# rrwick/Polypolish

Hardware: NVIDIA H100
Metric: assembly Mbp polished/sec (higher is better)
Workload: dtype u8 bases / u32 counters / f64 depth

## Files before the change

polypolish_b200/csrc/polish_dev.cuh:

```cuda
#pragma once

#include "nib_utils.h"
#include "../../include/pp_abi.h"

#define PP_BIN_SHIFT 8
#define PP_BIN (1u << PP_BIN_SHIFT)
#define PP_SUB_SHIFT 7
#define PP_SUB (1u << PP_SUB_SHIFT)
#define TL_T 2048
#define TL_THREADS 512
#define TL_PER_THREAD (TL_T / TL_THREADS)
#define TL_LONG_E 512
#define TL_QCAP 1024
#define TL_FAST_LEN 192
#define PR_THREADS 256
#define SC_GROUP_SCAN_LIMIT 8192
#define VT_THREADS 256
#define VT_ITEMS 8
#define VT_CHUNK (VT_THREADS * VT_ITEMS)
#define NONE32 0xFFFFFFFFu
static_assert(VT_CHUNK == TL_T, "k_tile hands k_compact one chunk per tile");
static_assert(TL_T % PP_BIN == 0 && TL_T / PP_SUB == TL_THREADS / 32 && TL_PER_THREAD * 32 == PP_SUB, "tile = whole bins; warp w owns depth sub-tile w and votes on it");

enum : unsigned {
    ERR_UNKNOWN_CONTIG = 1, ERR_SEQ_MISMATCH = 2, ERR_BAD_OP = 3, ERR_OOB = 4, ERR_NOSEQ = 5
};
enum : unsigned { FL_NODE_OVF = 1, FL_OUT_OVF = 8, FL_BIGGROUP = 16 };
enum : unsigned { TR_RC = 1, TR_FAST = 2, TR_LONG = 4, TR_FAST1 = 8 };

struct DevStatus {
    unsigned long long err;
    unsigned long long n_used;
    unsigned long long out_len;
    unsigned int node_count;
    unsigned int flags;
    unsigned int max_ext;
    unsigned int ticket;
    unsigned int n_changes;
    unsigned int pad1;
#ifdef PP_TILE_PROF
    unsigned long long prof[12];
#endif
};

struct DevParams {
    double fv, fi;
    uint32_t min_depth, max_errors;
    int careful;
    int pad;
};

struct OthNode {
    unsigned long long sig;
    unsigned long long val;
    uint32_t count;
    uint32_t next;
};

struct __align__(16) TileRec {
    uint32_t gstart;
    uint32_t seq_off;
    uint32_t cigar_off;
    uint32_t len_nc;
    uint32_t aln;
    uint32_t E;
    uint32_t flags;
    uint32_t cend;
};
#define TL_SEQ_QUADS 6

struct DevData {
    unsigned long long n_aln;
    const uint32_t *contig, *ref_start, *read_id, *seq_off, *cigar_off, *nm, *cigar_ops;
    const uint16_t *seq_len, *n_cigar;
// ... 575 lines not shown
    o.packed |= status << 26;
    if (vp.dbg) debug_record(vp.dbg + pos, depth, vt, it, cA, cC, cG, cT, cDel, matched, n_other, orig, status, o);
    if (CHG && status == 5) {
        const uint32_t slot = atomicAdd(vp.chg_n, 1u);
        if (slot < vp.chg_cap) {
            vp.chg_pos[slot] = pos;
            debug_record(vp.chg + slot, depth, vt, it, cA, cC, cG, cT, cDel, matched, n_other, orig, status, o);
        }
    }
    return o;
}

#define TL_DN_HALO 32
#define TL_INV_K 32
#define TL_DN_WORDS ((TL_T + 2 * TL_DN_HALO) / 16)

struct WalkStage {
    uint4 ent[64];
    uint32_t key[2][32];
};

#define TL_STAGES 2
struct ChunkStage {
    uint4 seq[32 * TL_SEQ_QUADS];
    TileRec rec[32];
};

#if defined(PP_EMULATE)
static inline void stage_bar_init(unsigned long long* bar) { emu::ring_init(bar); }
static inline void stage_fence() {}
static inline void stage_expect(unsigned long long* bar, uint32_t bytes) { emu::ring_expect(bar, bytes); }
static inline void stage_copy(void* dst, const void* src, uint32_t bytes, unsigned long long* bar) { emu::ring_copy(dst, src, bytes, bar); }
static inline void stage_wait(unsigned long long* bar, uint32_t parity) { emu::ring_wait(bar, parity); }
#else
__device__ __forceinline__ uint32_t smem_addr(const void* p) { return (uint32_t)__cvta_generic_to_shared(p); }
__device__ __forceinline__ void stage_bar_init(unsigned long long* bar) {
    asm volatile("mbarrier.init.shared::cta.b64 [%0], 1;\n\tfence.mbarrier_init.release.cluster;" ::"r"(smem_addr(bar)) : "memory");
}
__device__ __forceinline__ void stage_fence() { asm volatile("fence.proxy.async.shared::cta;" ::: "memory"); }
__device__ __forceinline__ void stage_expect(unsigned long long* bar, uint32_t bytes) {
    asm volatile("mbarrier.arrive.expect_tx.shared::cta.b64 _, [%0], %1;" ::"r"(smem_addr(bar)), "r"(bytes) : "memory");
}
__device__ __forceinline__ void stage_copy(void* dst, const void* src, uint32_t bytes, unsigned long long* bar) {
    asm volatile("cp.async.bulk.shared::cluster.global.mbarrier::complete_tx::bytes [%0], [%1], %2, [%3];"
                 ::"r"(smem_addr(dst)), "l"(src), "r"(bytes), "r"(smem_addr(bar)) : "memory");
}
__device__ __forceinline__ void stage_wait(unsigned long long* bar, uint32_t parity) {
    uint32_t done;
    do {
        asm volatile("{\n\t.reg .pred p;\n\tmbarrier.try_wait.parity.shared::cta.b64 p, [%1], %2;\n\tselp.u32 %0, 1, 0, p;\n\t}"
                     : "=r"(done) : "r"(smem_addr(bar)), "r"(parity) : "memory");
    } while (!done);
}
#endif

struct TileShared {
    int cdiff[TL_T + 4];
    uint32_t ex[4][TL_T];
    uint32_t del[TL_T];
    uint32_t oth[TL_T];
    union {
        unsigned long long deficit[TL_T + 4];
        double depth[TL_T];
    };
    unsigned long long dn[TL_DN_WORDS + 2];
    union {
        WalkStage wstage[TL_THREADS / 32];
        ChunkStage ring[TL_THREADS / 32][TL_STAGES];
    };
    unsigned long long ring_bar[TL_THREADS / 32][TL_STAGES];
    uint2 queue[TL_QCAP];
    uint32_t qn;
    unsigned long long s_warp[TL_THREADS / 32];
    unsigned long long s_total;
    long long s_delta[TL_THREADS / 32];
    uint32_t tile;
    uint32_t any_multi;
    double inv_k[TL_INV_K + 1];
    unsigned long long def_k[TL_INV_K + 1];
};
static_assert(sizeof(TileShared) <= 232448, "k_tile's shared memory: at most 227 KB per CTA on sm_90");

template <int BITS> struct TileCtx {
    const DevData& d;
    TileShared& sh;
    uint32_t P0;

    __device__ __forceinline__ bool in_tile(uint32_t pos) const { return pos - P0 < (uint32_t)TL_T; }
    __device__ __forceinline__ uint32_t draft_sym(uint32_t pos) const {
        if (BITS == 4) {
            const uint32_t o = pos - P0 + TL_DN_HALO;
            return (uint32_t)(sh.dn[o >> 4] >> ((o & 15) * 4)) & 15u;
        }
        const uint32_t b = d.draft[pos];
        return b == '-' ? 0u : b;
    }
    __device__ __forceinline__ void push_other(uint32_t pos, unsigned long long aln, uint32_t start, uint32_t len, unsigned long long sig) {
        if (!in_tile(pos)) return;
        atomicAdd(&sh.oth[pos - P0], 1u);
        other_insert<BITS>(d, pos, (aln << 32) | ((unsigned long long)(start & 0xFFFFu) << 16) | (len & 0xFFFFu), sig);
    }
    __device__ __forceinline__ void count_base(uint32_t pos, uint32_t s, unsigned long long aln, uint32_t ri) {
        if (!in_tile(pos)) return;
        if (Seq<BITS>::is_del(s)) { atomicAdd(&sh.del[pos - P0], 1u); return; }
        const uint32_t ds = draft_sym(pos);
// ... 18 lines not shown
    }
    __device__ __forceinline__ void scan_mismatches(unsigned long long r0, unsigned long long r1, uint32_t vc, uint32_t pos0,
                                                    unsigned long long aln, uint32_t ri0) {
        const long long rel64 = (long long)pos0 - (long long)P0;
        if (rel64 <= -32 || rel64 >= (long long)TL_T) return;
        const int rel0 = (int)rel64;
        unsigned long long d0, d1;
        draft32(rel0, d0, d1);
        unsigned long long m0, m1;
        mismatch_masks(r0, r1, d0, d1, vc, m0, m1);
        const int lo = -rel0, hi = TL_T - rel0;
        m0 &= nibmask(hi) & ~nibmask(lo);
        m1 &= nibmask(hi - 16) & ~nibmask(lo - 16);
        while (m0) {
            const uint32_t j = (uint32_t)(__ffsll((long long)m0) - 1) >> 2;
            m0 &= m0 - 1;
            const uint32_t code = (uint32_t)(r0 >> (4 * j)) & 15u;
            const int c = Seq<4>::acgt(code);
            if (c >= 0) atomicAdd(&sh.ex[c][rel0 + (int)j], 1u);
            else push_other(pos0 + j, aln, ri0 + j, 1, 1ull | ((unsigned long long)code << 4));
        }
        while (m1) {
            const uint32_t j = (uint32_t)(__ffsll((long long)m1) - 1) >> 2;
            m1 &= m1 - 1;
            const uint32_t code = (uint32_t)(r1 >> (4 * j)) & 15u;
            const int c = Seq<4>::acgt(code);
            if (c >= 0) atomicAdd(&sh.ex[c][rel0 + 16 + (int)j], 1u);
            else push_other(pos0 + 16 + j, aln, ri0 + 16 + j, 1, 1ull | ((unsigned long long)code << 4));
        }
    }
};

template <int BITS>
__device__ uint32_t general_walk(TileCtx<BITS>& S, const TileRec& r, uint32_t k) {
    const DevData& d = S.d;
    const unsigned long long aln = r.aln;
    const uint32_t len = r.len_nc & 0xFFFFu, ncig = r.len_nc >> 16;
    const bool rc = r.flags & TR_RC;
    const uint32_t gstart = r.gstart;
    const uint8_t* seqp = d.seq_pool + (size_t)r.seq_off * (BITS == 4 ? 16 : 32);
    const uint32_t* ops = d.cigar_ops + r.cigar_off;
    unsigned long long E = 0;
    for (uint32_t p = 0; p < ncig; ++p) {
        const uint32_t op = ops[p], o = op & 15u, l = op >> 4;
        if (o != PP_OP_I) E += l;
    }
    const uint32_t last = Seq<BITS>::read_sym(seqp, 0, len, rc, len - 1);
    unsigned long long run = 0;
    {
        uint32_t ri = len;
        uint32_t pend = 0;
        bool stop = false;
        for (int p = (int)ncig - 1; p >= 0 && !stop; --p) {
            const uint32_t op = ops[p], o = op & 15u, l = op >> 4;
            if (o == PP_OP_I) { pend += l; ri -= l; continue; }
            if (o == PP_OP_D) {
                for (uint32_t t = 0; t < l; ++t) {
                    if (pend == 1 && Seq<BITS>::read_sym(seqp, 0, len, rc, ri) == last) { run++; pend = 0; }
                    else { stop = true; break; }
                }
                continue;
            }
            for (uint32_t t = 0; t < l; ++t) {
                if (pend == 0 && Seq<BITS>::read_sym(seqp, 0, len, rc, ri - 1) == last) { run++; ri--; }
                else { stop = true; break; }
            }
        }
    }
    const unsigned long long nk64 = (E - run >= 1) ? (E - run - 1) : 0;
    if ((unsigned long long)gstart + nk64 > r.cend) { report_error(d.st, aln, ERR_OOB); return 0; }
    const uint32_t nkept = (uint32_t)nk64;
    S.add_interval(gstart, nkept, k);
    const long long off = (long long)S.P0 - (long long)gstart;
    const unsigned long long e_lo = off > 0 ? (unsigned long long)off : 0ull;
    const unsigned long long e_hi = min((unsigned long long)nkept, (unsigned long long)max(off + (long long)TL_T, 0ll));
    if (e_lo >= e_hi) return nkept;
    unsigned long long e = 0;
    uint32_t ri = 0;
    for (uint32_t p = 0; p < ncig && e < e_hi; ++p) {
        const uint32_t op = ops[p], o = op & 15u, l = op >> 4;
        if (o == PP_OP_I) { ri += l; continue; }
        uint32_t ins = 0;
        for (uint32_t q = p + 1; q < ncig && (ops[q] & 15u) == PP_OP_I; ++q) ins += ops[q] >> 4;
        const unsigned long long plain64 = min((unsigned long long)(ins ? l - 1 : l), (unsigned long long)nkept - e);
        const unsigned long long t_lo = e_lo > e ? e_lo - e : 0ull, t_hi = min(plain64, e_hi > e ? e_hi - e : 0ull);
        if (o == PP_OP_D) {
            for (unsigned long long t = t_lo; t < t_hi; ++t) atomicAdd(&S.sh.del[(uint32_t)(gstart + e + t) - S.P0], 1u);
            if (ins && e + l - 1 < nkept) {
                const uint32_t pos = (uint32_t)(gstart + e + l - 1);
                if (ins == 1) S.count_base(pos, Seq<BITS>::read_sym(seqp, 0, len, rc, ri), aln, ri);
                else S.push_other(pos, aln, ri, ins, make_sig<BITS>(seqp, 0, len, rc, ri, ins));
            }
            e += l;
            continue;
        }
        if (BITS == 4) {
            for (unsigned long long c0 = t_lo & ~31ull; c0 < t_hi; c0 += 32) {
                unsigned long long r0, r1;
                load_read32(reinterpret_cast<const unsigned long long*>(seqp), len, rc, ri + (uint32_t)c0, r0, r1);
                S.scan_mismatches(r0, r1, (uint32_t)min(plain64 - c0, 32ull), (uint32_t)(gstart + e + c0), aln, ri + (uint32_t)c0);
            }
        } else {
            for (unsigned long long t = t_lo; t < t_hi; ++t)
                S.count_base((uint32_t)(gstart + e + t), Seq<BITS>::read_sym(seqp, 0, len, rc, ri + (uint32_t)t), aln, ri + (uint32_t)t);
        }
        if (ins && e + l - 1 < nkept)
            S.push_other((uint32_t)(gstart + e + l - 1), aln, ri + l - 1, 1 + ins, make_sig<BITS>(seqp, 0, len, rc, ri + l - 1, 1 + ins));
        e += l;
        ri += l;
    }
    return nkept;
}

__device__ __forceinline__ uint32_t fast_walk(TileCtx<4>& S, const TileRec& r, const uint32_t* w, uint32_t k) {
    const uint32_t len = r.len_nc & 0xFFFFu;
    const unsigned long long aln = r.aln;
    if (len < 8) return NONE32;
    uint32_t run;
    const uint32_t tw = (len - 8) >> 3;
    const uint32_t tw0 = w[tw], tw1 = w[tw + 1];
    {
        const uint32_t o = len - 8;
        const uint32_t t8 = __funnelshift_r(tw0, tw1, (o & 7) * 4);
        const uint32_t x = t8 ^ ((t8 >> 28) * 0x11111111u);
        const uint32_t nz = (x | (x >> 1) | (x >> 2) | (x >> 3)) & 0x11111111u;
        if (nz == 0) return NONE32;
        run = 7u - ((31u - (uint32_t)__clz((int)nz)) >> 2);
    }
    const bool one = r.flags & TR_FAST1;
    const uint32_t ia = (r.flags >> 8) & 0xFFu, ib = (r.flags >> 16) & 0xFFFu;
    const bool is_del = (r.flags >> 28) & 1u;
    const uint32_t lc = len - ia - (is_del ? 0u : ib);
    if (run > lc) return NONE32;
    const uint32_t E = is_del ? len + ib : len - ib;
    const uint32_t nkept = E - run - 1;
    if ((unsigned long long)r.gstart + nkept > r.cend) { report_error(S.d.st, aln, ERR_OOB); return 0; }
    S.add_interval(r.gstart, nkept, k);
    const long long g0 = (long long)r.gstart - (long long)S.P0;
    if (g0 >= (long long)TL_T || g0 + (long long)nkept <= 0) return nkept;
    const uint32_t* dn32 = reinterpret_cast<const uint32_t*>(S.sh.dn);
    int relq[2], lo[2], hi[2], i0[2];
    uint32_t sh4[2], inner[2], edge[2];
    relq[0] = (int)g0;
    relq[1] = (int)g0 + (is_del ? (int)ib : -(int)ib);
    lo[0] = 0;
    hi[0] = !one ? (int)nkept : (int)ia - (is_del ? 0 : 1);
// ... 45 lines not shown
            const int rel = rq + 8 * (int)m + (int)t;
            if ((code & (code - 1)) == 0) atomicAdd(&S.sh.ex[__ffs((int)code) - 1][rel], 1u);
            else S.push_other(S.P0 + (uint32_t)rel, aln, 8u * m + t, 1, 1ull | ((unsigned long long)code << 4));
        }
    };
    uint32_t mm = (bits & cmp) | ((inner[0] | inner[1]) & ~cmp) | edge[0] | edge[1];
    {
        const bool sb = hi[1] > lo[1];
        const int e_lo = sb ? lo[1] : lo[0], e_hi = sb ? hi[1] : hi[0];
        const uint32_t m_last = (uint32_t)(e_hi - 1) >> 3;
        if (e_hi > e_lo && (((sb ? edge[1] : edge[0]) >> m_last) & 1u) && m_last - tw < 2u && (!sb || hi[0] <= 8 * (int)m_last)) {
            mm &= ~(1u << m_last);
            count_word(sb ? 1 : 0, m_last, m_last == tw ? tw0 : tw1);
        }
    }
    while (mm) {
        const uint32_t m = (uint32_t)__ffs((int)mm) - 1;
        mm &= mm - 1;
        const uint32_t wv = w[m];
        count_word(0, m, wv);
        if (one) count_word(1, m, wv);
    }
    if (one) {
        if (!is_del) {
            if (ia - 1 < nkept)
                S.push_other(r.gstart + ia - 1, aln, ia - 1, 1 + ib, make_sig<4>(S.d.seq_pool, r.seq_off, len, r.flags & TR_RC, ia - 1, 1 + ib));
        } else {
            const long long t0 = g0 + (long long)ia;
            const long long t_lo = max(0ll, -t0), t_hi = min((long long)min(ib, nkept - ia), (long long)TL_T - t0);
            for (long long t = t_lo; t < t_hi; ++t) atomicAdd(&S.sh.del[(int)(t0 + t)], 1u);
        }
    }
    return nkept;
}

__device__ __forceinline__ TileRec load_srec(const DevData& d, uint32_t slot) {
    const uint4* src = reinterpret_cast<const uint4*>(d.srec + slot);
    const uint4 a = __ldg(src), b = __ldg(src + 1);
    TileRec r;
    r.gstart = a.x; r.seq_off = a.y; r.cigar_off = a.z; r.len_nc = a.w; r.aln = b.x; r.E = b.y; r.flags = b.z; r.cend = b.w;
    return r;
}

#define DW_RUNS 4
#if defined(PP_EMULATE)
#define PP_PREFETCH_L1(p) ((void)(p))
#define PP_PREFETCH_L2(p) ((void)(p))
#else
#define PP_PREFETCH_L1(p) asm volatile("prefetch.global.L1 [%0];" ::"l"(p))
#define PP_PREFETCH_L2(p) asm volatile("prefetch.global.L2 [%0];" ::"l"(p))
#endif
template <int BITS>
__device__ void depth_walk_steps(const DevData& d, TileShared& sh, uint32_t P0, uint32_t sub, uint32_t lb, uint32_t long_lo, uint32_t long_hi) {
    const uint32_t lane = threadIdx.x & 31;
    const uint32_t s = P0 + sub * PP_SUB;
    const uint32_t bin = s >> PP_BIN_SHIFT;
    uint32_t wb[DW_RUNS], end[DW_RUNS], mask[DW_RUNS], head[DW_RUNS];
    uint32_t w_aln[DW_RUNS], w_start[DW_RUNS], w_len[DW_RUNS];
    double w_inv[DW_RUNS];
    auto load_window = [&](int r) {
        for (;;) {
            if (wb[r] >= end[r]) { mask[r] = 0; head[r] = NONE32; return; }
            const uint32_t slot = wb[r] + lane;
            uint4 q = make_uint4(NONE32, 0, 0, 1);
            if (slot < end[r]) {
                q = d.wrec[slot];
                if (slot + 32 < end[r]) PP_PREFETCH_L1(d.wrec + slot + 32);
            }
            uint32_t len = q.z;
            if (r == DW_RUNS - 1 && slot < end[r]) {
                const TileRec rec = load_srec(d, slot);
                const unsigned long long e_end = (unsigned long long)rec.gstart + rec.E;
                const uint32_t kk = d.kf[rec.aln];
                const bool mine = kk != 0 && e_end > P0 && rec.gstart < P0 + (uint32_t)TL_T;
                q.x = rec.aln; q.y = rec.gstart; q.w = mine ? kk : 1u;
                len = mine ? q.z : 0u;
// ... 122 lines not shown
    }
    double* out = sh.depth + (p - P0);
    out[0] = dep0; out[1] = dep1; out[2] = dep2; out[3] = dep3;
}

template <int BITS>
__device__ __forceinline__ void depth_walk(const DevData& d, TileShared& sh, WalkStage& ws, uint32_t P0, uint32_t sub, uint32_t lb, uint32_t long_lo, uint32_t long_hi) {
    const uint32_t bin = (P0 + sub * PP_SUB) >> PP_BIN_SHIFT;
    if (lb <= 1 && long_lo >= long_hi) {
        const uint32_t lo1 = d.bin_start[bin], hi1 = d.bin_start[bin + 1];
        uint32_t lo0 = 0, hi0 = 0;
        if (lb == 1 && bin >= 1) { lo0 = d.bin_start[bin - 1]; hi0 = lo1; }
        depth_walk_two<BITS>(d, sh, ws, P0, sub, lo0, hi0, lo1, hi1);
    } else depth_walk_steps<BITS>(d, sh, P0, sub, lb, long_lo, long_hi);
}

template <int BITS, bool CHG = false>
__device__ __forceinline__ void tile_body(const DevData& d, const VoteParams& vp, TileShared& sh) {
    const uint32_t tid = threadIdx.x, lane = tid & 31, warp = tid >> 5;
    const DevParams prm = *d.prm;
    const uint32_t lb = (d.max_ext + PP_BIN - 1) >> PP_BIN_SHIFT;
    const uint32_t long_lo = d.bin_start[d.n_bins], long_hi = d.bin_start[d.n_bins + 1];
    OthCtx oc;
    oc.nodes = d.nodes; oc.head = d.oth_head;
    oc.sr = SeqRef{d.seq_pool, d.seq_off, d.seq_len, d.flags};

    if (tid <= (uint32_t)TL_INV_K) {
        sh.inv_k[tid] = tid ? __ddiv_rn(1.0, (double)tid) : 0.0;
        sh.def_k[tid] = tid > 1 ? depth_deficit(tid) : 0ull;
    }
    ChunkStage* const ring = sh.ring[warp];
    unsigned long long* const bar = sh.ring_bar[warp];
    if (lane == 0) { stage_bar_init(&bar[0]); stage_bar_init(&bar[1]); }
    uint32_t parity = 0;
    for (;;) {
        stage_fence();
        __syncthreads();
        if (tid == 0) { sh.tile = atomicAdd(&d.st->ticket, 1u); sh.any_multi = 0; sh.qn = 0; }
        __syncthreads();
        if (sh.tile >= d.n_tiles) break;
        const uint32_t tile = d.tile_order[sh.tile];
        const uint32_t P0 = tile * (uint32_t)TL_T;
        TileCtx<BITS> S{d, sh, P0};
#ifdef PP_TILE_PROF
        long long pt[6];
        pt[0] = clock64();
#endif
        const uint32_t b0 = P0 >> PP_BIN_SHIFT;
        const uint32_t lo = d.bin_start[b0 >= lb ? b0 - lb : 0u];
        const uint32_t hi = d.bin_start[min(b0 + (uint32_t)(TL_T / PP_BIN), d.n_bins)];
        const uint32_t stride = 32u * (TL_THREADS / 32);
        uint32_t c_a = lo + 32u * warp;
        auto issue = [&](uint32_t c, uint32_t s) {
            const uint32_t n = min(32u, hi - c);
            stage_expect(&bar[s], n * (uint32_t)(sizeof(TileRec) + (BITS == 4 ? 16 * TL_SEQ_QUADS : 0)));
            stage_copy(ring[s].rec, d.srec + c, n * (uint32_t)sizeof(TileRec), &bar[s]);
            if (BITS == 4) stage_copy(ring[s].seq, d.sseq + (size_t)c * TL_SEQ_QUADS, n * 16u * TL_SEQ_QUADS, &bar[s]);
        };
        if (lane == 0) {
            if (c_a < hi) issue(c_a, 0);
            if (c_a + stride < hi) issue(c_a + stride, 1);
        }
        const uint32_t last_slot = d.n_slots ? d.n_slots - 1 : 0u;
        uint32_t k_a = 0;
        const uint32_t aln_a = __ldg(&d.srec[min(c_a + lane, last_slot)].aln);
        uint32_t aln_b = __ldg(&d.srec[min(c_a + stride + lane, last_slot)].aln);
        {
            uint4* z = reinterpret_cast<uint4*>(sh.cdiff);
            const uint32_t nz = (uint32_t)((size_t)((char*)sh.dn - (char*)sh.cdiff) / 16);
            for (uint32_t i = tid; i < nz; i += TL_THREADS) z[i] = make_uint4(0, 0, 0, 0);
            static_assert(TL_T == 4 * TL_THREADS, "one 16-byte store of chain heads per thread");
// ... 24 lines not shown
#ifdef PP_TILE_PROF
            unsigned long long wait_cyc = 0;
#endif
            uint32_t s = 0;
            while (c_a < hi) {
                const uint32_t c_b = c_a + stride, c_c = c_b + stride;
                uint32_t k_b = 0;
                if (c_b + lane < hi) k_b = d.kf[aln_b];
                const uint32_t aln_c = __ldg(&d.srec[min(c_c + lane, last_slot)].aln);
#ifdef PP_TILE_PROF
                const long long w0 = clock64();
#endif
                stage_wait(&bar[s], (parity >> s) & 1u);
                parity ^= 1u << s;
#ifdef PP_TILE_PROF
                if (lane == 0) wait_cyc += (unsigned long long)(clock64() - w0);
#endif
                const TileRec rec_a = ring[s].rec[lane];
                const uint32_t* const seq_a = reinterpret_cast<const uint32_t*>(ring[s].seq + lane * TL_SEQ_QUADS);
                const uint32_t i = c_a + lane;
                bool defer = false;
                if (i < hi) {
                    if (k_a == 0) d.wrec[i] = make_uint4(rec_a.aln, rec_a.gstart, 0u, 1u);
                    else {
                        uint32_t nk = NONE32;
                        if (BITS == 4 && (rec_a.flags & TR_FAST)) nk = fast_walk(reinterpret_cast<TileCtx<4>&>(S), rec_a, seq_a, k_a);
                        if (nk == NONE32) defer = true;
                        else d.wrec[i] = make_uint4(rec_a.aln, rec_a.gstart, nk, k_a);
                    }
                }
                if (defer) {
                    const uint32_t qi = atomicAdd(&sh.qn, 1u);
                    if (qi < TL_QCAP) {
                        sh.queue[qi] = make_uint2(i, k_a);
                        PP_PREFETCH_L2(d.cigar_ops + rec_a.cigar_off);
                        PP_PREFETCH_L2(d.seq_pool + (size_t)rec_a.seq_off * (BITS == 4 ? 16 : 32));
                    } else
                        d.wrec[i] = make_uint4(rec_a.aln, rec_a.gstart, general_walk<BITS>(S, rec_a, k_a), k_a);
                }
                __syncwarp();
                if (lane == 0 && c_c < hi) issue(c_c, s);
                c_a = c_b; aln_b = aln_c; k_a = k_b; s ^= 1u;
            }
#ifdef PP_TILE_PROF
            if (lane == 0 && wait_cyc) atomicAdd(&d.st->prof[11], wait_cyc);
#endif
        }
        __syncthreads();
#ifdef PP_TILE_PROF
        pt[2] = clock64();
#endif
        {
            const uint32_t qn = min(sh.qn, (uint32_t)TL_QCAP);
            for (uint32_t qi = lane * (TL_THREADS / 32) + warp; qi < qn; qi += TL_THREADS) {
                const uint2 q = sh.queue[qi];
                const TileRec r = load_srec(d, q.x);
                d.wrec[q.x] = make_uint4(r.aln, r.gstart, general_walk<BITS>(S, r, q.y), q.y);
            }
            for (uint32_t i = long_lo + tid; i < long_hi; i += TL_THREADS) {
                const TileRec r = load_srec(d, i);
                const unsigned long long e_end = (unsigned long long)r.gstart + r.E;
                const uint32_t k = d.kf[r.aln];
                if (k != 0 && e_end > P0 && r.gstart < P0 + (uint32_t)TL_T) d.wrec[i] = make_uint4(r.aln, r.gstart, general_walk<BITS>(S, r, k), k);
            }
        }
        __syncwarp();
        __syncthreads();
#ifdef PP_TILE_PROF
        pt[3] = clock64();
#endif
        const uint32_t rel0 = tid * TL_PER_THREAD;
        uint32_t cover[TL_PER_THREAD];
        uint32_t multi = 0;
        {
            long long csum = 0;
#pragma unroll
            for (int i = 0; i < TL_PER_THREAD; ++i) { csum += sh.cdiff[rel0 + i]; cover[i] = (uint32_t)csum; }
            const unsigned long long ex = block_exscan<TL_THREADS>((unsigned long long)csum, sh.s_warp, &sh.s_total);
#pragma unroll
            for (int i = 0; i < TL_PER_THREAD; ++i) cover[i] += (uint32_t)ex;
            if (sh.any_multi) {
                unsigned long long dsum = 0, dv[TL_PER_THREAD];
#pragma unroll
                for (int i = 0; i < TL_PER_THREAD; ++i) { dsum += sh.deficit[rel0 + i]; dv[i] = dsum; }
                const unsigned long long dex = block_exscan<TL_THREADS>(dsum, sh.s_warp, &sh.s_total);
#pragma unroll
                for (int i = 0; i < TL_PER_THREAD; ++i) {
                    sh.deficit[rel0 + i] = dv[i] + dex;
                    if (dv[i] + dex != 0 || cover[i] >= TL_DEF_COVER) multi |= 1u << i;
                }
            }
// ... 114 lines not shown
            if (n_zero) atomicAdd(&vp.zero_depth[ctg], (unsigned long long)n_zero);
            if (tdepth != 0.0) atomicAdd(&vp.total_depth[ctg], tdepth);
        }
        {
            uint32_t w2[TL_PER_THREAD / 2];
#pragma unroll
            for (int i = 0; i < TL_PER_THREAD; ++i) {
                const uint32_t len = po[i].packed & 0xFFFFu;
                uint32_t h;
                if ((po[i].packed >> 25) & 1u) { h = 255u << 8; if (p0 + i < d.G) vp.rec_at[p0 + i] = po[i].rec; }
                else h = (len << 8) | ((po[i].packed >> 16) & 255u);
                if (i & 1) w2[i >> 1] |= h << 16; else w2[i >> 1] = h;
            }
            *reinterpret_cast<uint2*>(vp.res + p0) = make_uint2(w2[0], w2[1]);
        }
        const uint32_t npos = (p0 < d.G) ? min((uint32_t)TL_PER_THREAD, d.G - p0) : 0u;
        long long delta = (long long)tlen - (long long)npos;
        for (int o = 16; o > 0; o >>= 1) delta += __shfl_down_sync(0xffffffffu, delta, o);
        if (lane == 0) sh.s_delta[warp] = delta;
#ifdef PP_TILE_PROF
        if (__syncthreads_or(walk) && tid == 0) atomicAdd(&d.st->prof[10], 1ull);
#endif
        __syncthreads();
        if (tid == 0) {
            long long t = 0;
            for (int i = 0; i < TL_THREADS / 32; ++i) t += sh.s_delta[i];
            vp.chunk_delta[tile] = t;
#ifdef PP_TILE_PROF
            pt[5] = clock64();
            for (int i = 0; i < 5; ++i) atomicAdd(&d.st->prof[i], (unsigned long long)(pt[i + 1] - pt[i]));
            atomicAdd(&d.st->prof[5], (unsigned long long)sh.qn);
            atomicAdd(&d.st->prof[6], 1ull);
            atomicMax(&d.st->prof[7], (unsigned long long)sh.qn);
#endif
        }
    }
}
static_assert(TL_PER_THREAD == 4, "the verdict store packs four positions per thread");

#if !defined(PP_EMULATE)
template <int BITS, bool CHG>
__global__ void __launch_bounds__(TL_THREADS, 1) k_tile(DevData d, VoteParams vp) {
    extern __shared__ __align__(16) unsigned char tile_smem[];
    tile_body<BITS, CHG>(d, vp, *reinterpret_cast<TileShared*>(tile_smem));
}
#endif

__device__ __forceinline__ uint8_t* put_u32(uint8_t* w, uint32_t v) {
    w[0] = (uint8_t)v; w[1] = (uint8_t)(v >> 8); w[2] = (uint8_t)(v >> 16); w[3] = (uint8_t)(v >> 24);
    return w + 4;
}
template <int BITS>
__device__ void allele_strings_row(const OthCtx& oc, uint32_t pos, uint32_t new_node, uint8_t* pool, unsigned long long cap,
                                   unsigned long long* used, unsigned long long* off) {
    unsigned long long bytes = 8;
    uint32_t n = 0;
    for (uint32_t nd = oc.head[pos]; nd != 0; nd = oc.nodes[nd - 1].next == NONE32 ? 0 : oc.nodes[nd - 1].next + 1) {
        bytes += 8 + ((uint32_t)oc.nodes[nd - 1].val & 0xFFFFu);
        n++;
    }
    const uint32_t new_len = new_node == NONE32 ? 0u : (uint32_t)oc.nodes[new_node].val & 0xFFFFu;
    bytes += new_len;
    const unsigned long long o = atomicAdd(used, bytes);
    *off = o;
    if (o + bytes > cap) return;
    uint8_t* w = put_u32(pool + o, n);
// ... 126 lines not shown
```

polypolish_b200/csrc/polish_kernels.cu:

```cuda
#include <cuda_runtime.h>

#include <cub/device/device_radix_sort.cuh>
#include <cub/device/device_scan.cuh>

#include <algorithm>
#include <functional>
#include <cstddef>
#include <cstdio>
#include <string>
#include <vector>

#include "pp_internal.h"
#include "pp_ctx.cuh"
#include "polish_dev.cuh"


static void init_comp_table(uint8_t* t) {
    for (int i = 0; i < 256; ++i) t[i] = 'N';
    const char* a = "ATGCNRYSWKMBVDH.-?";
    const char* b = "TACGNYRSWMKVBHD.-?";
    for (int i = 0; a[i]; ++i) t[(unsigned char)a[i]] = (uint8_t)b[i];
}

extern "C" const char* pp_version(void) { return "0.6.1-b200"; }
// ... 399 lines not shown
        vp.res = ctx->b[B_RES].as<uint16_t>(); vp.rec_at = ctx->b[B_RECAT].as<uint32_t>();
        vp.chunk_delta = ctx->b[B_CHUNKDELTA].as<long long>();
        vp.dbg = nullptr;
        if (ctx->debug_on) { CK(ctx->b[B_DEBUG].ensure((G + 1) * sizeof(pp_debug_pos))); vp.dbg = ctx->b[B_DEBUG].as<pp_debug_pos>(); }
        vp.chg = nullptr; vp.chg_pos = nullptr; vp.chg_n = &d.st->n_changes; vp.chg_cap = 0;
        if (ctx->changes_on) {
            if (ctx->chg_cap == 0) ctx->chg_cap = (uint32_t)std::max<uint64_t>(4096, G / 256);
            CK(ctx->b[B_CHG].ensure((size_t)ctx->chg_cap * sizeof(pp_debug_pos))); CK(ctx->b[B_CHGPOS].ensure((size_t)ctx->chg_cap * 4));
            vp.chg = ctx->b[B_CHG].as<pp_debug_pos>(); vp.chg_pos = ctx->b[B_CHGPOS].as<uint32_t>(); vp.chg_cap = ctx->chg_cap;
        }
        {
            int occ = 1;
            CK(cudaOccupancyMaxActiveBlocksPerMultiprocessor(&occ, vp.chg ? k_tile<BITS, true> : k_tile<BITS, false>, TL_THREADS, sizeof(TileShared)));
            const uint32_t grid = std::min<uint32_t>(n_tiles, (uint32_t)ctx->sm_count * (uint32_t)std::max(occ, 1));
            if (vp.chg) k_tile<BITS, true><<<grid, TL_THREADS, sizeof(TileShared), s>>>(d, vp);
            else k_tile<BITS, false><<<grid, TL_THREADS, sizeof(TileShared), s>>>(d, vp);
            ctx->launches++;
        }
        CK(cudaEventRecord(ctx->ev[4], s));
        k_compact<BITS><<<n_tiles, VT_THREADS, 0, s>>>(d, vp);
        ctx->launches++;
        CK(cudaEventRecord(ctx->ev[5], s));
        CK(cudaMemcpyAsync(ctx->h_status, d.st, sizeof(DevStatus), cudaMemcpyDeviceToHost, s));
        CK(cudaStreamSynchronize(s));
        CK(cudaGetLastError());
        const DevStatus hs = *ctx->h_status;
#ifdef PP_TILE_PROF
        fprintf(stderr, "[tile prof] tiles %llu; cycles/tile: A %.0f B %.0f queue %.0f C %.0f D+E %.0f; queued reads/tile %.1f (max %llu); "
                "chunk wait/tile/warp %.0f\n", hs.prof[6],
                (double)hs.prof[0] / hs.prof[6], (double)hs.prof[1] / hs.prof[6], (double)hs.prof[2] / hs.prof[6], (double)hs.prof[3] / hs.prof[6],
                (double)hs.prof[4] / hs.prof[6], (double)hs.prof[5] / hs.prof[6], hs.prof[7], (double)hs.prof[11] / hs.prof[6] / (TL_THREADS / 32));
        fprintf(stderr, "[tile prof] depth walks %llu (%.2f per tile, %llu tiles with one), %.0f cycles each\n", hs.prof[9], (double)hs.prof[9] / hs.prof[6], hs.prof[10],
                hs.prof[9] ? (double)hs.prof[8] / hs.prof[9] : 0.0);
#endif
        if (hs.err != ~0ull) {
            res->error_aln = (int64_t)(hs.err >> 8);
            return ctx->fail(PP_ERR_INPUT, std::string(err_text((unsigned)(hs.err & 0xFF))) + " (alignment " + std::to_string(hs.err >> 8) + ")");
        }
        bool again = false;
        if (hs.flags & FL_BIGGROUP) { if (ctx->global_k) return ctx->fail(PP_ERR_CUDA, "internal error: FL_BIGGROUP in global-k mode"); ctx->global_k = true; again = true; }
        if (hs.flags & FL_NODE_OVF) { ctx->node_cap = (uint32_t)std::min<uint64_t>(0x7FFFFFFFull, (uint64_t)hs.node_count + hs.node_count / 4 + 1024); again = true; }
        if (!again && (hs.flags & FL_OUT_OVF)) { ctx->out_cap = hs.out_len + 64; again = true; }
        if (!again && ctx->changes_on && hs.n_changes > ctx->chg_cap) { ctx->chg_cap = hs.n_changes; again = true; }
        if (again) continue;

        ctx->have_debug = ctx->debug_on; ctx->last_head = d.oth_head; ctx->last_nodes = std::min(hs.node_count, node_cap);
        ctx->have_changes = ctx->changes_on; ctx->n_changes = ctx->changes_on ? hs.n_changes : 0; ctx->chg_pool = -1;
        res->out_len = hs.out_len;
        res->n_aln_used = hs.n_used;
        res->error_aln = -1;
        memset(&res->timing, 0, sizeof res->timing);
        float ms;
        CK(cudaEventElapsedTime(&ms, ctx->ev[0], ctx->ev[1])); res->timing.stage_ms[0] = ms;
        CK(cudaEventElapsedTime(&ms, ctx->ev[1], ctx->ev[2])); res->timing.stage_ms[1] = ms;
        CK(cudaEventElapsedTime(&ms, ctx->ev[2], ctx->ev[3])); res->timing.stage_ms[2] = ms;
        CK(cudaEventElapsedTime(&ms, ctx->ev[3], ctx->ev[4])); res->timing.stage_ms[3] = ms;
        CK(cudaEventElapsedTime(&ms, ctx->ev[4], ctx->ev[5])); res->timing.stage_ms[4] = ms;
        CK(cudaEventElapsedTime(&ms, ctx->ev[0], ctx->ev[5])); res->timing.total_ms = ms;
        res->timing.launches = ctx->launches;

        if (res->out_bases) {
            if (res->out_cap < hs.out_len) return ctx->fail(PP_ERR_ARG, "out_cap too small: need " + std::to_string(hs.out_len) + " bytes");
            CK(cudaEventRecord(ctx->ev[7], s));
            CK(cudaMemcpyAsync(res->out_bases, vp.out, hs.out_len, cudaMemcpyDeviceToHost, s));
            if (res->out_off) CK(cudaMemcpyAsync(res->out_off, vp.out_off, ((size_t)ctx->n_contigs + 1) * 8, cudaMemcpyDeviceToHost, s));
            if (res->changed) CK(cudaMemcpyAsync(res->changed, vp.changed, (size_t)ctx->n_contigs * 8, cudaMemcpyDeviceToHost, s));
// ... 172 lines not shown
```

Before: 8319.

## Drain deferred-read queue with early-finishing warps and stage walks in shared memory

Warps that finish the chunk loop early now pull deferred reads from a shared work queue using CAS and acquire loads while other warps are still busy, instead of waiting at the barrier. Each queued walk copies the read's sequence and CIGAR into the warp's free ring buffer in shared memory before lane 0 walks it, which cuts global-memory latency during the serial walk. This adds spin-wait and nanosleep overhead, a fence, and more atomics on shared memory. It also adds extra profiling counters.

```diff
diff --git a/polypolish_b200/csrc/polish_dev.cuh b/polypolish_b200/csrc/polish_dev.cuh
--- a/polypolish_b200/csrc/polish_dev.cuh
+++ b/polypolish_b200/csrc/polish_dev.cuh
@@ -39,7 +39,7 @@
     unsigned int n_changes;
     unsigned int pad1;
 #ifdef PP_TILE_PROF
-    unsigned long long prof[12];
+    unsigned long long prof[17];
 #endif
 };
 
@@ -681,7 +681,14 @@
 static inline void stage_expect(unsigned long long* bar, uint32_t bytes) { emu::ring_expect(bar, bytes); }
 static inline void stage_copy(void* dst, const void* src, uint32_t bytes, unsigned long long* bar) { emu::ring_copy(dst, src, bytes, bar); }
 static inline void stage_wait(unsigned long long* bar, uint32_t parity) { emu::ring_wait(bar, parity); }
+template <class V> static inline V ld_acquire_cta(const V* p) { return __atomic_load_n(p, __ATOMIC_ACQUIRE); }
+static inline void st_relaxed_cta(unsigned long long* p, unsigned long long v) { __atomic_store_n(p, v, __ATOMIC_RELAXED); }
+static inline void fence_cta() { std::atomic_thread_fence(std::memory_order_seq_cst); }
+static inline void backoff(unsigned ns) { std::this_thread::sleep_for(std::chrono::nanoseconds(ns)); }
+static std::atomic<unsigned long long> emu_queue_walks[3];
+#define EMU_QUEUE_COUNT(i, n) emu_queue_walks[i].fetch_add(n)
 #else
+#define EMU_QUEUE_COUNT(i, n) ((void)0)
 __device__ __forceinline__ uint32_t smem_addr(const void* p) { return (uint32_t)__cvta_generic_to_shared(p); }
 __device__ __forceinline__ void stage_bar_init(unsigned long long* bar) {
     asm volatile("mbarrier.init.shared::cta.b64 [%0], 1;\n\tfence.mbarrier_init.release.cluster;" ::"r"(smem_addr(bar)) : "memory");
@@ -701,6 +708,21 @@
                      : "=r"(done) : "r"(smem_addr(bar)), "r"(parity) : "memory");
     } while (!done);
 }
+__device__ __forceinline__ uint32_t ld_acquire_cta(const uint32_t* p) {
+    uint32_t v;
+    asm volatile("ld.acquire.cta.shared::cta.u32 %0, [%1];" : "=r"(v) : "r"(smem_addr(p)) : "memory");
+    return v;
+}
+__device__ __forceinline__ unsigned long long ld_acquire_cta(const unsigned long long* p) {
+    unsigned long long v;
+    asm volatile("ld.acquire.cta.shared::cta.u64 %0, [%1];" : "=l"(v) : "r"(smem_addr(p)) : "memory");
+    return v;
+}
+__device__ __forceinline__ void st_relaxed_cta(unsigned long long* p, unsigned long long v) {
+    asm volatile("st.relaxed.cta.shared::cta.u64 [%0], %1;" ::"r"(smem_addr(p)), "l"(v) : "memory");
+}
+__device__ __forceinline__ void fence_cta() { __threadfence_block(); }
+__device__ __forceinline__ void backoff(unsigned ns) { __nanosleep(ns); }
 #endif
 
 struct TileShared {
@@ -718,8 +740,11 @@
         ChunkStage ring[TL_THREADS / 32][TL_STAGES];
     };
     unsigned long long ring_bar[TL_THREADS / 32][TL_STAGES];
-    uint2 queue[TL_QCAP];
-    uint32_t qn;
+    unsigned long long queue[TL_QCAP];
+    uint32_t qn, take, warps_done;
+#ifdef PP_TILE_PROF
+    unsigned long long leave_lo, leave_hi;
+#endif
     unsigned long long s_warp[TL_THREADS / 32];
     unsigned long long s_total;
     long long s_delta[TL_THREADS / 32];
@@ -804,14 +829,12 @@
 };
 
 template <int BITS>
-__device__ uint32_t general_walk(TileCtx<BITS>& S, const TileRec& r, uint32_t k) {
+__device__ uint32_t general_walk(TileCtx<BITS>& S, const TileRec& r, uint32_t k, const uint32_t* ops, const uint8_t* seqp) {
     const DevData& d = S.d;
     const unsigned long long aln = r.aln;
     const uint32_t len = r.len_nc & 0xFFFFu, ncig = r.len_nc >> 16;
     const bool rc = r.flags & TR_RC;
     const uint32_t gstart = r.gstart;
-    const uint8_t* seqp = d.seq_pool + (size_t)r.seq_off * (BITS == 4 ? 16 : 32);
-    const uint32_t* ops = d.cigar_ops + r.cigar_off;
     unsigned long long E = 0;
     for (uint32_t p = 0; p < ncig; ++p) {
         const uint32_t op = ops[p], o = op & 15u, l = op >> 4;
@@ -883,6 +906,10 @@
     }
     return nkept;
 }
+template <int BITS>
+__device__ __forceinline__ uint32_t general_walk(TileCtx<BITS>& S, const TileRec& r, uint32_t k) {
+    return general_walk<BITS>(S, r, k, S.d.cigar_ops + r.cigar_off, S.d.seq_pool + (size_t)r.seq_off * (BITS == 4 ? 16 : 32));
+}
 
 __device__ __forceinline__ uint32_t fast_walk(TileCtx<4>& S, const TileRec& r, const uint32_t* w, uint32_t k) {
     const uint32_t len = r.len_nc & 0xFFFFu;
@@ -1005,6 +1032,39 @@
     return r;
 }
 
+#define TL_STAGE_BYTES (TL_STAGES * (uint32_t)sizeof(ChunkStage))
+template <int BITS>
+__device__ __forceinline__ void stage_walk(TileCtx<BITS>& S, ChunkStage* stage, uint32_t slot, uint32_t k) {
+    const DevData& d = S.d;
+    const uint32_t lane = threadIdx.x & 31;
+    const TileRec r = load_srec(d, slot);
+    const uint32_t len = r.len_nc & 0xFFFFu, ncig = r.len_nc >> 16;
+    const uint32_t nq = (len + 31) / 32 * (BITS == 4 ? 1u : 2u);
+    const uint4* gq = reinterpret_cast<const uint4*>(d.seq_pool + (size_t)r.seq_off * (BITS == 4 ? 16 : 32));
+    const uint32_t* gops = d.cigar_ops + r.cigar_off;
+    uint32_t nk = 0;
+    if (16u * (nq + 1) + 4u * ncig <= TL_STAGE_BYTES) {
+        uint4* sq = reinterpret_cast<uint4*>(stage);
+        uint32_t* sops = reinterpret_cast<uint32_t*>(sq + nq + 1);
+        for (uint32_t i = lane; i <= nq; i += 32) sq[i] = i < nq ? gq[i] : make_uint4(0, 0, 0, 0);
+        for (uint32_t i = lane; i < ncig; i += 32) sops[i] = gops[i];
+        __syncwarp();
+        if (lane == 0) {
+#ifdef PP_TILE_PROF
+            const long long t0 = clock64();
+#endif
+            nk = general_walk<BITS>(S, r, k, sops, reinterpret_cast<const uint8_t*>(sq));
+            EMU_QUEUE_COUNT(2, 1);
+#ifdef PP_TILE_PROF
+            atomicAdd(&d.st->prof[14], (unsigned long long)(clock64() - t0));
+            atomicAdd(&d.st->prof[15], 1ull);
+#endif
+        }
+        __syncwarp();
+    } else if (lane == 0) nk = general_walk<BITS>(S, r, k, gops, reinterpret_cast<const uint8_t*>(gq));
+    if (lane == 0) d.wrec[slot] = make_uint4(r.aln, r.gstart, nk, k);
+}
+
 #define DW_RUNS 4
 #if defined(PP_EMULATE)
 #define PP_PREFETCH_L1(p) ((void)(p))
@@ -1193,11 +1253,17 @@
     ChunkStage* const ring = sh.ring[warp];
     unsigned long long* const bar = sh.ring_bar[warp];
     if (lane == 0) { stage_bar_init(&bar[0]); stage_bar_init(&bar[1]); }
+    for (uint32_t i = tid; i < (uint32_t)TL_QCAP; i += TL_THREADS) sh.queue[i] = 0;
     uint32_t parity = 0;
     for (;;) {
         stage_fence();
         __syncthreads();
-        if (tid == 0) { sh.tile = atomicAdd(&d.st->ticket, 1u); sh.any_multi = 0; sh.qn = 0; }
+        if (tid == 0) {
+            sh.tile = atomicAdd(&d.st->ticket, 1u); sh.any_multi = 0; sh.qn = 0; sh.take = 0; sh.warps_done = 0;
+#ifdef PP_TILE_PROF
+            sh.leave_lo = ~0ull; sh.leave_hi = 0;
+#endif
+        }
         __syncthreads();
         if (sh.tile >= d.n_tiles) break;
         const uint32_t tile = d.tile_order[sh.tile];
@@ -1288,7 +1354,7 @@
                 if (defer) {
                     const uint32_t qi = atomicAdd(&sh.qn, 1u);
                     if (qi < TL_QCAP) {
-                        sh.queue[qi] = make_uint2(i, k_a);
+                        st_relaxed_cta(&sh.queue[qi], (unsigned long long)k_a << 32 | i);
                         PP_PREFETCH_L2(d.cigar_ops + rec_a.cigar_off);
                         PP_PREFETCH_L2(d.seq_pool + (size_t)rec_a.seq_off * (BITS == 4 ? 16 : 32));
                     } else
@@ -1302,17 +1368,65 @@
             if (lane == 0 && wait_cyc) atomicAdd(&d.st->prof[11], wait_cyc);
 #endif
         }
+        __syncwarp();
+        if (lane == 0) {
+#ifdef PP_TILE_PROF
+            const unsigned long long now = (unsigned long long)clock64();
+            atomicMin(&sh.leave_lo, now);
+            atomicMax(&sh.leave_hi, now);
+#endif
+            fence_cta();
+            atomicAdd(&sh.warps_done, 1u);
+        }
+        for (;;) {
+            uint32_t qi = NONE32;
+            unsigned long long q = 0;
+            if (lane == 0) {
+                for (;;) {
+                    if (ld_acquire_cta(&sh.warps_done) == TL_THREADS / 32) break;
+                    const uint32_t n = min(ld_acquire_cta(&sh.qn), (uint32_t)TL_QCAP), t = ld_acquire_cta(&sh.take);
+                    if (t < n) {
+                        if (atomicCAS(&sh.take, t, t + 1u) == t) { qi = t; break; }
+                    } else backoff(128);
+                }
+                if (qi != NONE32) {
+                    while (((q = ld_acquire_cta(&sh.queue[qi])) >> 32) == 0) backoff(32);
+                    sh.queue[qi] = 0;
+                }
+            }
+            q = __shfl_sync(0xffffffffu, q, 0);
+            if (q == 0) break;
+            stage_walk<BITS>(S, ring, (uint32_t)q, (uint32_t)(q >> 32));
+            if (lane == 0) EMU_QUEUE_COUNT(0, 1);
+#ifdef PP_TILE_PROF
+            if (lane == 0) atomicAdd(&d.st->prof[12], 1ull);
+#endif
+        }
         __syncthreads();
 #ifdef PP_TILE_PROF
         pt[2] = clock64();
 #endif
         {
-            const uint32_t qn = min(sh.qn, (uint32_t)TL_QCAP);
-            for (uint32_t qi = lane * (TL_THREADS / 32) + warp; qi < qn; qi += TL_THREADS) {
-                const uint2 q = sh.queue[qi];
-                const TileRec r = load_srec(d, q.x);
-                d.wrec[q.x] = make_uint4(r.aln, r.gstart, general_walk<BITS>(S, r, q.y), q.y);
-            }
+            const uint32_t qn = min(sh.qn, (uint32_t)TL_QCAP), q0 = sh.take;
+            if (qn - q0 <= TL_THREADS / 32) {
+                if (q0 + warp < qn) {
+                    const unsigned long long q = sh.queue[q0 + warp];
+                    __syncwarp();
+                    if (lane == 0) sh.queue[q0 + warp] = 0;
+                    stage_walk<BITS>(S, ring, (uint32_t)q, (uint32_t)(q >> 32));
+                }
+            } else {
+                for (uint32_t qi = q0 + lane * (TL_THREADS / 32) + warp; qi < qn; qi += TL_THREADS) {
+                    const unsigned long long q = sh.queue[qi];
+                    sh.queue[qi] = 0;
+                    const TileRec r = load_srec(d, (uint32_t)q);
+                    d.wrec[(uint32_t)q] = make_uint4(r.aln, r.gstart, general_walk<BITS>(S, r, (uint32_t)(q >> 32)), (uint32_t)(q >> 32));
+                }
+            }
+            if (tid == 0) EMU_QUEUE_COUNT(1, qn - q0);
+#ifdef PP_TILE_PROF
+            if (tid == 0) atomicAdd(&d.st->prof[13], (unsigned long long)(qn - q0));
+#endif
             for (uint32_t i = long_lo + tid; i < long_hi; i += TL_THREADS) {
                 const TileRec r = load_srec(d, i);
                 const unsigned long long e_end = (unsigned long long)r.gstart + r.E;
@@ -1493,6 +1607,7 @@
             atomicAdd(&d.st->prof[5], (unsigned long long)sh.qn);
             atomicAdd(&d.st->prof[6], 1ull);
             atomicMax(&d.st->prof[7], (unsigned long long)sh.qn);
+            atomicAdd(&d.st->prof[16], sh.leave_hi - sh.leave_lo);
 #endif
         }
     }
diff --git a/polypolish_b200/csrc/polish_kernels.cu b/polypolish_b200/csrc/polish_kernels.cu
--- a/polypolish_b200/csrc/polish_kernels.cu
+++ b/polypolish_b200/csrc/polish_kernels.cu
@@ -455,6 +455,9 @@
                 (double)hs.prof[4] / hs.prof[6], (double)hs.prof[5] / hs.prof[6], hs.prof[7], (double)hs.prof[11] / hs.prof[6] / (TL_THREADS / 32));
         fprintf(stderr, "[tile prof] depth walks %llu (%.2f per tile, %llu tiles with one), %.0f cycles each\n", hs.prof[9], (double)hs.prof[9] / hs.prof[6], hs.prof[10],
                 hs.prof[9] ? (double)hs.prof[8] / hs.prof[9] : 0.0);
+        fprintf(stderr, "[tile prof] queued reads/tile walked during B %.2f, after it %.2f; %.0f cycles per staged walk (%llu); warps leave the chunk "
+                "loop over %.0f cycles/tile\n", (double)hs.prof[12] / hs.prof[6], (double)hs.prof[13] / hs.prof[6],
+                hs.prof[15] ? (double)hs.prof[14] / hs.prof[15] : 0.0, hs.prof[15], (double)hs.prof[16] / hs.prof[6]);
 #endif
         if (hs.err != ~0ull) {
             res->error_aln = (int64_t)(hs.err >> 8);
```

Measured after the change: 8382, median of 6. About the same (+0.8%).

## Walk queued general alignments with a whole warp instead of one thread

Applied to the files above, without the earlier changes.

For 4-bit sequences, queued general-walk alignments are now processed one per warp rather than one per thread. Lanes cooperatively prefix-scan CIGAR op lengths, detect the trailing homopolymer run with a mismatch mask, and distribute 32-base chunks of match/deletion spans across lanes. This replaces serial per-thread CIGAR walks that caused warp divergence and load imbalance in the queue phase. It adds shuffle/scan overhead per alignment and falls back to the serial path for zero-length ops; profiling counters are extended too.

```diff
diff --git a/polypolish_b200/csrc/polish_dev.cuh b/polypolish_b200/csrc/polish_dev.cuh
--- a/polypolish_b200/csrc/polish_dev.cuh
+++ b/polypolish_b200/csrc/polish_dev.cuh
@@ -39,7 +39,7 @@
     unsigned int n_changes;
     unsigned int pad1;
 #ifdef PP_TILE_PROF
-    unsigned long long prof[12];
+    unsigned long long prof[16];
 #endif
 };
 
@@ -804,6 +804,30 @@
 };
 
 template <int BITS>
+__device__ unsigned long long trim_run(const uint8_t* seqp, uint32_t len, bool rc, const uint32_t* ops, uint32_t ncig) {
+    const uint32_t last = Seq<BITS>::read_sym(seqp, 0, len, rc, len - 1);
+    unsigned long long run = 0;
+    uint32_t ri = len;
+    uint32_t pend = 0;
+    for (int p = (int)ncig - 1; p >= 0; --p) {
+        const uint32_t op = ops[p], o = op & 15u, l = op >> 4;
+        if (o == PP_OP_I) { pend += l; ri -= l; continue; }
+        if (o == PP_OP_D) {
+            for (uint32_t t = 0; t < l; ++t) {
+                if (pend == 1 && Seq<BITS>::read_sym(seqp, 0, len, rc, ri) == last) { run++; pend = 0; }
+                else return run;
+            }
+            continue;
+        }
+        for (uint32_t t = 0; t < l; ++t) {
+            if (pend == 0 && Seq<BITS>::read_sym(seqp, 0, len, rc, ri - 1) == last) { run++; ri--; }
+            else return run;
+        }
+    }
+    return run;
+}
+
+template <int BITS>
 __device__ uint32_t general_walk(TileCtx<BITS>& S, const TileRec& r, uint32_t k) {
     const DevData& d = S.d;
     const unsigned long long aln = r.aln;
@@ -817,28 +841,7 @@
         const uint32_t op = ops[p], o = op & 15u, l = op >> 4;
         if (o != PP_OP_I) E += l;
     }
-    const uint32_t last = Seq<BITS>::read_sym(seqp, 0, len, rc, len - 1);
-    unsigned long long run = 0;
-    {
-        uint32_t ri = len;
-        uint32_t pend = 0;
-        bool stop = false;
-        for (int p = (int)ncig - 1; p >= 0 && !stop; --p) {
-            const uint32_t op = ops[p], o = op & 15u, l = op >> 4;
-            if (o == PP_OP_I) { pend += l; ri -= l; continue; }
-            if (o == PP_OP_D) {
-                for (uint32_t t = 0; t < l; ++t) {
-                    if (pend == 1 && Seq<BITS>::read_sym(seqp, 0, len, rc, ri) == last) { run++; pend = 0; }
-                    else { stop = true; break; }
-                }
-                continue;
-            }
-            for (uint32_t t = 0; t < l; ++t) {
-                if (pend == 0 && Seq<BITS>::read_sym(seqp, 0, len, rc, ri - 1) == last) { run++; ri--; }
-                else { stop = true; break; }
-            }
-        }
-    }
+    const unsigned long long run = trim_run<BITS>(seqp, len, rc, ops, ncig);
     const unsigned long long nk64 = (E - run >= 1) ? (E - run - 1) : 0;
     if ((unsigned long long)gstart + nk64 > r.cend) { report_error(d.st, aln, ERR_OOB); return 0; }
     const uint32_t nkept = (uint32_t)nk64;
@@ -884,6 +887,158 @@
     return nkept;
 }
 
+__device__ __forceinline__ TileRec load_srec(const DevData& d, uint32_t slot) {
+    const uint4* src = reinterpret_cast<const uint4*>(d.srec + slot);
+    const uint4 a = __ldg(src), b = __ldg(src + 1);
+    TileRec r;
+    r.gstart = a.x; r.seq_off = a.y; r.cigar_off = a.z; r.len_nc = a.w; r.aln = b.x; r.E = b.y; r.flags = b.z; r.cend = b.w;
+    return r;
+}
+
+__device__ __forceinline__ uint32_t warp_incl_scan(uint32_t v) {
+    const int lane = (int)(threadIdx.x & 31);
+    for (int o = 1; o < 32; o <<= 1) {
+        const uint32_t t = __shfl_up_sync(0xffffffffu, v, o);
+        if (lane >= o) v += t;
+    }
+    return v;
+}
+
+__device__ __forceinline__ void walk_op_end(TileCtx<4>& S, const uint8_t* seqp, uint32_t len, bool rc, unsigned long long aln, uint32_t gstart,
+                                            uint32_t nkept, bool is_del, uint32_t e, uint32_t ri_end, uint32_t ins) {
+    const uint32_t pos = gstart + e;
+    if (e >= nkept || !S.in_tile(pos)) return;
+    if (is_del) {
+        if (ins == 0) atomicAdd(&S.sh.del[pos - S.P0], 1u);
+        else if (ins == 1) S.count_base(pos, Seq<4>::read_sym(seqp, 0, len, rc, ri_end), aln, ri_end);
+        else S.push_other(pos, aln, ri_end, ins, make_sig<4>(seqp, 0, len, rc, ri_end, ins));
+    } else {
+        if (ins == 0) S.count_base(pos, Seq<4>::read_sym(seqp, 0, len, rc, ri_end - 1), aln, ri_end - 1);
+        else S.push_other(pos, aln, ri_end - 1, 1 + ins, make_sig<4>(seqp, 0, len, rc, ri_end - 1, 1 + ins));
+    }
+}
+
+__device__ __forceinline__ uint32_t general_walk_warp(TileCtx<4>& S, uint32_t slot, uint32_t k) {
+    const DevData& d = S.d;
+    const uint32_t lane = threadIdx.x & 31;
+    const TileRec r = load_srec(d, slot);
+    const unsigned long long aln = r.aln;
+    const uint32_t len = r.len_nc & 0xFFFFu, ncig = r.len_nc >> 16;
+    const bool rc = r.flags & TR_RC;
+    const uint32_t gstart = r.gstart;
+    const uint8_t* seqp = d.seq_pool + (size_t)r.seq_off * 16;
+    const unsigned long long* seq64 = reinterpret_cast<const unsigned long long*>(seqp);
+    const uint32_t* ops = d.cigar_ops + r.cigar_off;
+    const uint32_t op_first = lane < ncig ? ops[lane] : (uint32_t)PP_OP_I;
+    const uint32_t op_last = ops[ncig - 1];
+    unsigned long long x0 = 0, x1 = 0;
+    if (lane == 0) load_read32(seq64, len, rc, len > 32 ? len - 32 : 0u, x0, x1);
+    uint32_t E = 0;
+    bool zero = false;
+    for (uint32_t base = 0; base < ncig; base += 32) {
+        const uint32_t p = base + lane;
+        const uint32_t op = base == 0 ? op_first : (p < ncig ? ops[p] : (uint32_t)PP_OP_I);
+        uint32_t el = (op & 15u) != PP_OP_I ? op >> 4 : 0u;
+        zero |= __ballot_sync(0xffffffffu, p < ncig && (op >> 4) == 0) != 0;
+        el = warp_incl_scan(el);
+        E += __shfl_sync(0xffffffffu, el, 31);
+    }
+    uint32_t nkept;
+    if (zero) {
+        uint32_t nk = 0;
+        if (lane == 0) nk = general_walk<4>(S, r, k);
+        nkept = __shfl_sync(0xffffffffu, nk, 0);
+        if (lane == 0) d.wrec[slot] = make_uint4(r.aln, gstart, nkept, k);
+        return nkept;
+    }
+    uint32_t run;
+    {
+        uint32_t h = NONE32;
+        if (lane == 0) {
+            const uint32_t n = min(len, 32u);
+            const unsigned long long last = ((n <= 16 ? x0 >> (4 * (n - 1)) : x1 >> (4 * (n - 17))) & 15ull) * 0x1111111111111111ull;
+            unsigned long long m0, m1;
+            mismatch_masks(x0, x1, last, last, n, m0, m1);
+            if (m0 | m1) h = n - 1 - (uint32_t)((m1 ? 64 + 63 - __clzll((long long)m1) : 63 - __clzll((long long)m0)) >> 2);
+        }
+        h = __shfl_sync(0xffffffffu, h, 0);
+        const uint32_t ol = op_last & 15u;
+        if ((ol == PP_OP_M || ol == PP_OP_EQ || ol == PP_OP_X) && h < (op_last >> 4)) run = h;
+        else {
+            uint32_t rr = 0;
+            if (lane == 0) rr = (uint32_t)trim_run<4>(seqp, len, rc, ops, ncig);
+            run = __shfl_sync(0xffffffffu, rr, 0);
+        }
+    }
+    nkept = E - run >= 1 ? E - run - 1 : 0u;
+    if ((unsigned long long)gstart + nkept > r.cend) {
+        if (lane == 0) { report_error(d.st, aln, ERR_OOB); d.wrec[slot] = make_uint4(r.aln, gstart, 0u, k); }
+        return 0;
+    }
+    if (lane == 0) { S.add_interval(gstart, nkept, k); d.wrec[slot] = make_uint4(r.aln, gstart, nkept, k); }
+    const long long off = (long long)S.P0 - (long long)gstart;
+    const uint32_t e_lo = off > 0 ? (uint32_t)off : 0u;
+    const uint32_t e_hi = (uint32_t)min((long long)nkept, max(off + (long long)TL_T, 0ll));
+    if (e_lo >= e_hi) return nkept;
+    uint32_t e_c = 0, ri_c = 0;
+    bool pend = false, pend_del = false;
+    uint32_t pend_e = 0, pend_ri = 0;
+    for (uint32_t base = 0; base < ncig; base += 32) {
+        const uint32_t p = base + lane;
+        const uint32_t op = base == 0 ? op_first : (p < ncig ? ops[p] : (uint32_t)PP_OP_I);
+        const uint32_t o = op & 15u, l = op >> 4;
+        const bool non_i = o != PP_OP_I, is_del = o == PP_OP_D;
+        const uint32_t el = non_i ? l : 0u, rl = is_del ? 0u : l;
+        const uint32_t ei = warp_incl_scan(el), rin = warp_incl_scan(rl);
+        const uint32_t e0 = e_c + ei - el, r0 = ri_c + rin - rl;
+        const uint32_t ri_w = ri_c + __shfl_sync(0xffffffffu, rin, 31);
+        const uint32_t nim = __ballot_sync(0xffffffffu, non_i);
+        const uint32_t after = nim & ~((2u << lane) - 1u);
+        const uint32_t r_next = __shfl_sync(0xffffffffu, r0, after ? __ffs((int)after) - 1 : (int)lane);
+        if (pend && nim) {
+            const uint32_t r_first = __shfl_sync(0xffffffffu, r0, __ffs((int)nim) - 1);
+            if (lane == 0) walk_op_end(S, seqp, len, rc, aln, gstart, nkept, pend_del, pend_e, pend_ri, r_first - pend_ri);
+            pend = false;
+        }
+        const bool last_window = base + 32 >= ncig;
+        if (non_i && (after || last_window))
+            walk_op_end(S, seqp, len, rc, aln, gstart, nkept, is_del, e0 + l - 1, r0 + rl, (after ? r_next : ri_w) - (r0 + rl));
+        if (!last_window && nim) {
+            const int L = 31 - __clz((int)nim);
+            const uint32_t le = __shfl_sync(0xffffffffu, e0 + l - 1, L), lri = __shfl_sync(0xffffffffu, r0 + rl, L);
+            const bool ld = __shfl_sync(0xffffffffu, is_del ? 1u : 0u, L) != 0;
+            pend = true; pend_del = ld; pend_e = le; pend_ri = lri;
+        }
+        const uint32_t b_lo = max(e0, e_lo), b_hi2 = non_i ? min(e0 + l - 1, e_hi) : 0u;
+        const uint32_t np = b_hi2 > b_lo ? (b_hi2 - b_lo + 31) / 32 : 0u;
+        const uint32_t pin = warp_incl_scan(np), pex = pin - np, NP = __shfl_sync(0xffffffffu, pin, 31);
+        for (uint32_t pb = 0; pb < NP; pb += 32) {
+            const uint32_t pi = pb + lane;
+            uint32_t j = 0;
+            for (uint32_t s = 16; s; s >>= 1) if (__shfl_sync(0xffffffffu, pex, (int)(j + s)) <= pi) j += s;
+            const uint32_t jlo = __shfl_sync(0xffffffffu, b_lo, (int)j), jhi = __shfl_sync(0xffffffffu, b_hi2, (int)j);
+            const uint32_t jpex = __shfl_sync(0xffffffffu, pex, (int)j), je0 = __shfl_sync(0xffffffffu, e0, (int)j);
+            const uint32_t jr0 = __shfl_sync(0xffffffffu, r0, (int)j);
+            const bool jdel = __shfl_sync(0xffffffffu, is_del ? 1u : 0u, (int)j) != 0;
+            if (pi < NP) {
+                const uint32_t s0 = jlo + 32 * (pi - jpex), vc = min(32u, jhi - s0);
+                if (jdel) {
+                    for (uint32_t t = 0; t < vc; ++t) atomicAdd(&S.sh.del[gstart + s0 + t - S.P0], 1u);
+                } else {
+                    const uint32_t ri = jr0 + (s0 - je0);
+                    unsigned long long q0, q1;
+                    load_read32(seq64, len, rc, ri, q0, q1);
+                    S.scan_mismatches(q0, q1, vc, gstart + s0, aln, ri);
+                }
+            }
+        }
+        e_c += __shfl_sync(0xffffffffu, ei, 31);
+        ri_c = ri_w;
+    }
+    if (pend && lane == 0) walk_op_end(S, seqp, len, rc, aln, gstart, nkept, pend_del, pend_e, pend_ri, ri_c - pend_ri);
+    return nkept;
+}
+
 __device__ __forceinline__ uint32_t fast_walk(TileCtx<4>& S, const TileRec& r, const uint32_t* w, uint32_t k) {
     const uint32_t len = r.len_nc & 0xFFFFu;
     const unsigned long long aln = r.aln;
@@ -995,14 +1150,6 @@
         }
     }
     return nkept;
-}
-
-__device__ __forceinline__ TileRec load_srec(const DevData& d, uint32_t slot) {
-    const uint4* src = reinterpret_cast<const uint4*>(d.srec + slot);
-    const uint4 a = __ldg(src), b = __ldg(src + 1);
-    TileRec r;
-    r.gstart = a.x; r.seq_off = a.y; r.cigar_off = a.z; r.len_nc = a.w; r.aln = b.x; r.E = b.y; r.flags = b.z; r.cend = b.w;
-    return r;
 }
 
 #define DW_RUNS 4
@@ -1308,10 +1455,23 @@
 #endif
         {
             const uint32_t qn = min(sh.qn, (uint32_t)TL_QCAP);
-            for (uint32_t qi = lane * (TL_THREADS / 32) + warp; qi < qn; qi += TL_THREADS) {
-                const uint2 q = sh.queue[qi];
-                const TileRec r = load_srec(d, q.x);
-                d.wrec[q.x] = make_uint4(r.aln, r.gstart, general_walk<BITS>(S, r, q.y), q.y);
+            if constexpr (BITS == 4) {
+                for (uint32_t qi = warp; qi < qn; qi += TL_THREADS / 32) {
+                    const uint2 q = sh.queue[qi];
+#ifdef PP_TILE_PROF
+                    const long long g0 = clock64();
+#endif
+                    general_walk_warp(reinterpret_cast<TileCtx<4>&>(S), q.x, q.y);
+#ifdef PP_TILE_PROF
+                    if (tid == 0) { atomicAdd(&d.st->prof[14], (unsigned long long)(clock64() - g0)); atomicAdd(&d.st->prof[15], 1ull); }
+#endif
+                }
+            } else {
+                for (uint32_t qi = lane * (TL_THREADS / 32) + warp; qi < qn; qi += TL_THREADS) {
+                    const uint2 q = sh.queue[qi];
+                    const TileRec r = load_srec(d, q.x);
+                    d.wrec[q.x] = make_uint4(r.aln, r.gstart, general_walk<BITS>(S, r, q.y), q.y);
+                }
             }
             for (uint32_t i = long_lo + tid; i < long_hi; i += TL_THREADS) {
                 const TileRec r = load_srec(d, i);
@@ -1493,6 +1653,7 @@
             atomicAdd(&d.st->prof[5], (unsigned long long)sh.qn);
             atomicAdd(&d.st->prof[6], 1ull);
             atomicMax(&d.st->prof[7], (unsigned long long)sh.qn);
+            if (sh.qn == 0) { atomicAdd(&d.st->prof[12], (unsigned long long)(pt[3] - pt[2])); atomicAdd(&d.st->prof[13], 1ull); }
 #endif
         }
     }
diff --git a/polypolish_b200/csrc/polish_kernels.cu b/polypolish_b200/csrc/polish_kernels.cu
--- a/polypolish_b200/csrc/polish_kernels.cu
+++ b/polypolish_b200/csrc/polish_kernels.cu
@@ -455,6 +455,13 @@
                 (double)hs.prof[4] / hs.prof[6], (double)hs.prof[5] / hs.prof[6], hs.prof[7], (double)hs.prof[11] / hs.prof[6] / (TL_THREADS / 32));
         fprintf(stderr, "[tile prof] depth walks %llu (%.2f per tile, %llu tiles with one), %.0f cycles each\n", hs.prof[9], (double)hs.prof[9] / hs.prof[6], hs.prof[10],
                 hs.prof[9] ? (double)hs.prof[8] / hs.prof[9] : 0.0);
+        {
+            const unsigned long long t0 = hs.prof[13], t1 = hs.prof[6] - hs.prof[13];
+            fprintf(stderr, "[tile prof] queue cycles/tile: %.0f in %llu tiles without a queued read, %.0f in %llu tiles with one; "
+                            "thread 0's queued general walks %llu, %.0f cycles each\n",
+                    t0 ? (double)hs.prof[12] / t0 : 0.0, t0, t1 ? (double)(hs.prof[2] - hs.prof[12]) / t1 : 0.0, t1, hs.prof[15],
+                    hs.prof[15] ? (double)hs.prof[14] / hs.prof[15] : 0.0);
+        }
 #endif
         if (hs.err != ~0ull) {
             res->error_aln = (int64_t)(hs.err >> 8);
```

After: 8303 before, 8463 after, median of 6. 1.02x the previous value.
